# michaelriedl/2048-ppo-agent

Hardware: AMD Instinct MI355X
Metric: env-steps/sec at N parallel boards (full PPO loop: rollout with policy in the loop + GAE + update) (higher is better)
Workload: dtype u8 boards / bf16 policy; 1 GPU; 65536 parallel boards per GPU, Transformer policy bf16 (3.96 M params), full PPO iteration (BASELINE.json configs[2]; configs[3] when n_gpus=8); boards_per_gpu=65536, global_boards=65536, train_batch=2048, update_epochs=5, max_samples_per_epoch=300000, max_samples_per_epoch_is=global (each rank draws its 1/N share), as the reference's single subset, max_samples_per_epoch_per_rank=300000, rollout_mode=episodes (reference lock-step semantics), rng_mode=partitionable, parallelism=env-shard x1 + 1 grad all-reduce/minibatch

## Files before the change

2048-ppo-agent_amd/csrc/g2048_policy.hip:

```cpp
#include <hip/hip_runtime.h>
#include <stddef.h>
#include <stdint.h>
#include <stdlib.h>

#include "../../include/g2048.h"
#include "g2048_host.h"
#include "g2048_mfma.h"

namespace {

using g2048_mfma::bf16x4;
using g2048_mfma::bf16x8;
using g2048_mfma::f32x16;
using g2048_mfma::f32x4;
using g2048_mfma::mfma;
using g2048_mfma::rowof;
using g2048_mfma::sched_fence;
using g2048_mfma::static_for;
using namespace g2048_host;

typedef short s16x2 __attribute__((ext_vector_type(2)));

constexpr int D = 256, NH = 8, HD = 32, FF = 1024, SEQ = 17, NBOARD = 7, NTOK = 128, THREADS = 256;
constexpr int W_LAYER = 3 * D * D + D * D + FF * D + D * FF;
constexpr int P_LAYER = D + D + 3 * D + D + D + D + FF + D;
constexpr int WO_QKV = 0, WO_O = 3 * D * D, WO_1 = WO_O + D * D, WO_2 = WO_1 + FF * D;
constexpr int PO_LN1G = 0, PO_LN1B = D, PO_BQKV = 2 * D, PO_BO = 5 * D, PO_LN2G = 6 * D, PO_LN2B = 7 * D,
              PO_B1 = 8 * D, PO_B2 = 8 * D + FF;
constexpr int FFC = 64;
constexpr int TILE = 32 * D * 2;
constexpr float SM_SCALE_LOG2E = 0.17677669529663687f * 1.4426950408889634f;

template <int CPR> __device__ __forceinline__ int swz(int r);
template <> __device__ __forceinline__ int swz<32>(int r) { return r & 15; }
template <> __device__ __forceinline__ int swz<16>(int r) { return r & 15; }
template <> __device__ __forceinline__ int swz<8>(int r) { return (r >> 1) & 7; }
template <> __device__ __forceinline__ int swz<4>(int r) { return (r >> 2) & 3; }

struct LaneOff {
    int a256[8];
    int a64[4];
    int a32[2];
    unsigned s256[2], s64, s32;
};
__device__ __forceinline__ void lane_offsets(LaneOff &o, int r, int h, int w, int lane) {
    for (int k = 0; k < 8; ++k) o.a256[k] = r * 512 + (((2 * k + h) ^ swz<32>(r)) * 16);
    for (int k = 0; k < 4; ++k) o.a64[k] = r * 128 + (((2 * k + h) ^ swz<8>(r)) * 16);
    for (int k = 0; k < 2; ++k) o.a32[k] = r * 64 + (((2 * k + h) ^ swz<4>(r)) * 16);
    for (int par = 0; par < 2; ++par) {
        const int x = 2 * w + (lane >> 5), row15 = (8 * par + x) & 15;
        o.s256[par] = (unsigned)(x * D * 2 + (((lane & 31) ^ row15) * 16));
    }
    {
        const int x = 8 * w + (lane >> 3);
        o.s64 = (unsigned)(x * FF * 2 + (((lane & 7) ^ swz<8>(x)) * 16));
    }
    {
        const int x = 16 * w + (lane >> 2);
        o.s32 = (unsigned)(x * D * 2 + (((lane & 3) ^ swz<4>(x)) * 16));
    }
}

template <int CPR>
__device__ __forceinline__ bf16x8 load_w(const char *tile, const LaneOff &o, int mt, int ks) {
    if (CPR == 32) return *reinterpret_cast<const bf16x8 *>(tile + o.a256[ks & 7] + (ks >> 3) * 256 + mt * 32 * 512);
    if (CPR == 8) return *reinterpret_cast<const bf16x8 *>(tile + o.a64[ks] + mt * 32 * 128);
    return *reinterpret_cast<const bf16x8 *>(tile + o.a32[ks] + mt * 32 * 64);
}
__device__ __forceinline__ bf16x8 load_p(const char *row, int ks, int h) {
    return *reinterpret_cast<const bf16x8 *>(row + 2 * (16 * ks + 8 * h));
}

__device__ __forceinline__ void frag_from_acc(const f32x16 &x, bf16x8 out[2]) {
    for (int s = 0; s < 2; ++s)
        for (int j = 0; j < 8; ++j) out[s][j] = (__bf16)x[8 * s + j];
}
__device__ __forceinline__ void relu_frag_from_acc(const f32x16 &x, bf16x8 out[2]) {
    frag_from_acc(x, out);
    for (int s = 0; s < 2; ++s) {
        s16x2 *p = reinterpret_cast<s16x2 *>(&out[s]);
        const s16x2 zero = {0, 0};
        for (int q = 0; q < 4; ++q) p[q] = __builtin_elementwise_max(p[q], zero);
    }
}

__device__ __forceinline__ f32x16 bias_tile(const float *b32, int h) {
    f32x16 a;
    for (int g = 0; g < 4; ++g) {
        const f32x4 v = *reinterpret_cast<const f32x4 *>(b32 + 8 * g + 4 * h);
        for (int q = 0; q < 4; ++q) a[4 * g + q] = v[q];
    }
    return a;
}

template <int CPR, int NK, bool SWAP = false>
__device__ __forceinline__ f32x16 gemm_tile(const char *tile, const LaneOff &o, int mt, const bf16x8 *b, f32x16 acc) {
    bf16x8 a[NK];
    for (int ks = 0; ks < NK; ++ks) a[ks] = load_w<CPR>(tile, o, mt, ks);
    for (int ks = 0; ks < NK; ++ks) acc = SWAP ? mfma(b[ks], a[ks], acc) : mfma(a[ks], b[ks], acc);
    return acc;
}
template <int NM, int EXTRA = 0, int NV = 0, int VALU_PER = 0, int TRANS_PER = 0, int DEPTH = 8>
__device__ __forceinline__ void pipe_mfma() {
    __builtin_amdgcn_sched_group_barrier(0x100, DEPTH + EXTRA, 0);
#pragma unroll
    for (int i = 0; i < NM; ++i) {
        __builtin_amdgcn_sched_group_barrier(0x008, 1, 0);
        if (i < NM - DEPTH) __builtin_amdgcn_sched_group_barrier(0x100, 1, 0);
        if (i < NV && VALU_PER) __builtin_amdgcn_sched_group_barrier(0x002, VALU_PER, 0);
        if (i < NV && TRANS_PER) __builtin_amdgcn_sched_group_barrier(0x400, TRANS_PER, 0);
    }
}

#ifdef G2048_STAMPS
constexpr int N_STAMPS = 24;
__device__ unsigned long long g_stamps[N_STAMPS];
struct StampSite {
    __device__ __forceinline__ static bool on(int lane, int w) { return lane == 0 && w == 0 && blockIdx.x % 64 == 0; }
    __device__ __forceinline__ static unsigned long long *table(int) { return g_stamps; }
};
#define STAMP(k) stamps.mark(k)
#else
#define STAMP(k)
#endif

typedef __amdgpu_buffer_rsrc_t rsrc_t;
template <int CPR>
__device__ __forceinline__ void dma_tile(char *dst, rsrc_t blob, unsigned src_byte, int ld, int rows, const LaneOff &o, int w) {
    const int n_inst = rows * CPR / (64 * 4);
    const int rows_per_inst = 4 * 64 / CPR;
    for (int t = 0; t < n_inst; ++t) {
        const unsigned lane_off = CPR == 32 ? o.s256[t & 1] : (CPR == 8 ? o.s64 : o.s32);
        __builtin_amdgcn_raw_ptr_buffer_load_lds(blob, (__attribute__((address_space(3))) void *)(dst + (t * 4 + w) * 1024), 16,
                                                 (int)lane_off, (int)(src_byte + (unsigned)(t * rows_per_inst * ld * 2)), 0, 0);
    }
}
template <int CPR>
__device__ __forceinline__ void dma_inst(char *dst, rsrc_t blob, unsigned src_byte, int ld, int t, const LaneOff &o, int w) {
    const int rows_per_inst = 4 * 64 / CPR;
    const unsigned lane_off = CPR == 32 ? o.s256[t & 1] : (CPR == 8 ? o.s64 : o.s32);
    __builtin_amdgcn_raw_ptr_buffer_load_lds(blob, (__attribute__((address_space(3))) void *)(dst + (t * 4 + w) * 1024), 16,
                                             (int)lane_off, (int)(src_byte + (unsigned)(t * rows_per_inst * ld * 2)), 0, 0);
}
template <int N> __device__ __forceinline__ void dma_wait() { asm volatile("s_waitcnt vmcnt(%0)" ::"n"(N) : "memory"); }
__device__ __forceinline__ void dma_wait_all() { dma_wait<0>(); }

__device__ __forceinline__ void stage_f32(float *dst, const float *src, int n, int tid) {
    for (int i = tid; i < n; i += THREADS) dst[i] = src[i];
}

__device__ __forceinline__ void park_in_agpr(bf16x8 &x) { asm volatile("" : "+a"(x)); }

__device__ __forceinline__ float xhalf_sum(float x) {
    const auto r = __builtin_amdgcn_permlane32_swap(__float_as_uint(x), __float_as_uint(x), false, false);
    return __uint_as_float(r[0]) + __uint_as_float(r[1]);
}
__device__ __forceinline__ float xhalf_max(float x) {
    const auto r = __builtin_amdgcn_permlane32_swap(__float_as_uint(x), __float_as_uint(x), false, false);
    return fmaxf(__uint_as_float(r[0]), __uint_as_float(r[1]));
}

__device__ __forceinline__ void layer_norm(const f32x16 r[8], bf16x8 out[16]) {
    typedef float f32x2 __attribute__((ext_vector_type(2)));
    f32x2 s2[4], q2[4];
    for (int k = 0; k < 4; ++k) s2[k] = q2[k] = f32x2{0.f, 0.f};
    for (int j = 0; j < 8; ++j)
        for (int i = 0; i < 16; i += 2) {
            const f32x2 v = {r[j][i], r[j][i + 1]};
            const int k = (i >> 1) & 3;
            s2[k] += v;
            q2[k] = __builtin_elementwise_fma(v, v, q2[k]);
        }
    const f32x2 st = (s2[0] + s2[1]) + (s2[2] + s2[3]), qt = (q2[0] + q2[1]) + (q2[2] + q2[3]);
    float s = st[0] + st[1], ss = qt[0] + qt[1];
    s = xhalf_sum(s);
    ss = xhalf_sum(ss);
    const float mean = s * (1.0f / D);
    const float var = fmaxf(__builtin_fmaf(-mean, mean, ss * (1.0f / D)), 0.0f);
    const float rstd = rsqrtf(var + 1e-5f), shift = -mean * rstd;
    for (int j = 0; j < 8; ++j)
        for (int i = 0; i < 16; ++i) out[2 * j + (i >> 3)][i & 7] = (__bf16)__builtin_fmaf(r[j][i], rstd, shift);
    for (int k = 0; k < 16; ++k) park_in_agpr(out[k]);
}

constexpr int MODE_FULL = 0, MODE_HEAD = 1, MODE_MEAN = 2, MODE_CLS = 3;
constexpr int64_t KV_ELEMS = (int64_t)NH * SEQ * HD;

constexpr int L_WQKV = 0;
constexpr int L_WO = 6 * TILE;
constexpr int L_K = 7 * TILE;
constexpr int L_VT = 7 * TILE + TILE / 2;
constexpr int L_W1 = 0;
constexpr int L_W2 = 4 * TILE;
constexpr int L_CX = 6 * TILE;
constexpr int L_CQ = L_CX + 4096;
constexpr int L_CS = L_CQ + 1024;
constexpr int L_CO = L_CS + 1280;
constexpr int L_CV = 7 * TILE;
static_assert(L_CO + (NBOARD + 1) * D * 2 <= L_CV && L_CV + 2 * NTOK * HD * 2 <= 8 * TILE, "CLS staging fits the free tiles");
struct LdsMain {
    char w[8 * TILE];
    float bq[D], bo[D], b1[FF], b2[D];
};
static_assert(sizeof(LdsMain) <= 160 * 1024, "LDS budget");
constexpr int MEAN_LD = D + 4;
static_assert(NBOARD * 16 * MEAN_LD * 4 <= (int)sizeof(LdsMain::w), "mean-pool stage fits over the weight area");

template <int MODE>
__global__ void __launch_bounds__(THREADS, 1)
k_encoder_main(const uint8_t *__restrict__ boards, const float *__restrict__ table, const float *__restrict__ cls,
               const __bf16 *__restrict__ wblob, const float *__restrict__ pblob, int n_layers,
               float *__restrict__ features, int64_t B, __bf16 *__restrict__ ws_k, __bf16 *__restrict__ ws_v,
               float *__restrict__ ws_r) {
    extern __shared__ __attribute__((aligned(16))) char smem[];
    LdsMain &L = *reinterpret_cast<LdsMain *>(smem);
    const int tid = threadIdx.x, lane = tid & 63, r = lane & 31, h = lane >> 5;
    const int w = __builtin_amdgcn_readfirstlane(tid >> 6);
    const int64_t board0 = (int64_t)blockIdx.x * NBOARD;
    LaneOff lo;
    lane_offsets(lo, r, h, w, lane);

    const int tok = 32 * w + r;
    const int tb = tok / SEQ;
    const int tc = tok - tb * SEQ;
    const bool tok_valid = tb < NBOARD && board0 + tb < B;

    const int kb = w == 0 ? 0 : (w == 1 ? 16 : (w == 2 ? 48 : 64));
    int k_rd[2], vt_rd[4], k_wr[2], vt_wr[2];
    for (int ks = 0; ks < 2; ++ks) k_rd[ks] = L_K + kb * 64 + lo.a32[ks];
    for (int ks = 0; ks < 4; ++ks) vt_rd[ks] = L_VT + r * 256 + (((kb / 8 + 2 * ks + h) ^ swz<16>(r)) * 16);
    for (int s = 0; s < 2; ++s) {
        k_wr[s] = L_K + tok * 64 + (((2 * s + h) ^ swz<4>(tok)) * 16);
        vt_wr[s] = L_VT + r * 256 + (((4 * w + 2 * s + h) ^ swz<16>(r)) * 16);
    }
    bf16x8 kmask[2], qmask;
    {
        const int qb = tb;
        for (int j = 0; j < 8; ++j) qmask[j] = (__bf16)((qb == 8 * h + j) ? 16.0f : 0.0f);
        for (int tl = 0; tl < 2; ++tl) {
            const int kbd = (kb + 32 * tl + r) / SEQ;
            for (int j = 0; j < 8; ++j) kmask[tl][j] = (__bf16)((kbd == 8 * h + j) ? 16.0f : 0.0f);
        }
        park_in_agpr(qmask);
        park_in_agpr(kmask[0]);
        park_in_agpr(kmask[1]);
    }

    f32x16 R[8];
    {
        const float *src = cls;
        if (tok_valid && tc != 0) {
            int e = boards[(board0 + tb) * 16 + (tc - 1)];
            e = e > 30 ? 30 : e;
            src = table + ((size_t)(tc - 1) * 31 + e) * D;
        }
        const float keep = tok_valid ? 1.0f : 0.0f;
        for (int j = 0; j < 8; ++j)
            for (int g = 0; g < 4; ++g) {
                const f32x4 v = *reinterpret_cast<const f32x4 *>(src + 32 * j + 8 * g + 4 * h);
                for (int q = 0; q < 4; ++q) R[j][4 * g + q] = keep * v[q];
            }
    }

    const int full_layers = (MODE == MODE_HEAD || MODE == MODE_CLS) ? n_layers - 1 : n_layers;
    char *const lds = L.w;
    const rsrc_t blob = __builtin_amdgcn_make_buffer_rsrc(const_cast<__bf16 *>(wblob), 0, n_layers * (W_LAYER * 2), 0x00020000);
    auto wqkv = [&](int hd) -> char * { return lds + L_WQKV + (hd & 1) * 3 * TILE; };
    auto dma_qkv1 = [&](unsigned lw, int hd, int n) __attribute__((always_inline)) {
        dma_inst<32>(wqkv(hd) + (n / 4) * TILE, blob, lw + 2u * (unsigned)(WO_QKV + ((n / 4) * D + HD * hd) * D), D, n % 4, lo, w);
    };
    auto dma_wo1 = [&](unsigned lw, int hd, int n) __attribute__((always_inline)) {
        dma_inst<4>(lds + L_WO, blob, lw + 2u * (unsigned)(WO_O + HD * hd), D, n, lo, w);
    };
    auto dma_w11 = [&](unsigned lw, int c, int n) __attribute__((always_inline)) {
        dma_inst<32>(lds + L_W1 + (c & 1) * 2 * TILE, blob, lw + 2u * (unsigned)(WO_1 + FFC * c * D), D, n, lo, w);
    };
    auto dma_w21 = [&](unsigned lw, int c, int n) __attribute__((always_inline)) {
        dma_inst<8>(lds + L_W2 + (c & 1) * 2 * TILE, blob, lw + 2u * (unsigned)(WO_2 + FFC * c), FF, n, lo, w);
    };

#ifdef G2048_STAMPS
    g2048_mfma::Stamps<N_STAMPS, StampSite> stamps;
    stamps.start();
#endif
    for (int n = 0; n < 12; ++n) dma_qkv1(0u, 0, n);
    for (int n = 0; n < 12; ++n) dma_qkv1(0u, 1, n);

    constexpr int PD = 8;
    bf16x8 xn[16];
#pragma nounroll
    for (int layer = 0; layer < full_layers; ++layer) {
        const unsigned lw = (unsigned)layer * (unsigned)(W_LAYER * 2);
        const float *P = pblob + (size_t)layer * P_LAYER;

        float stg[7];
        stg[0] = P[PO_BQKV + tid];
        stg[1] = P[PO_BO + tid];
        stg[2] = P[PO_B2 + tid];
        for (int q = 0; q < 4; ++q) stg[3 + q] = P[PO_B1 + 256 * q + tid];
        layer_norm(R, xn);
        L.bq[tid] = stg[0];
        L.bo[tid] = stg[1];
        L.b2[tid] = stg[2];
        for (int q = 0; q < 4; ++q) L.b1[256 * q + tid] = stg[3 + q];
        dma_wait_all();
        __syncthreads();
        STAMP(0);

        f32x16 qa, ka, va;
        bf16x8 qf[2], kf[2], vf[2];
        auto project = [&](int hd, auto softmax_tag, auto fetch, f32x16 &s0, f32x16 &s1, bf16x8 *pf, float &sum) __attribute__((always_inline)) {
            constexpr bool SOFTMAX = decltype(softmax_tag)::value;
            const char *t = wqkv(hd);
            bf16x8 a[PD];
            qa = bias_tile(L.bq + HD * hd, h);
            for (int i = 0; i < 16; ++i) ka[i] = va[i] = 0.f;
            static_for<0, PD>([&](auto ic) __attribute__((always_inline)) {
                constexpr int i = decltype(ic)::value;
                a[i] = load_w<32>(t + (i / 16) * TILE, lo, 0, i % 16);
            });
            float m = 0.f, mc = 0.f;
            sched_fence();
            static_for<0, 48>([&](auto ic) __attribute__((always_inline)) {
                constexpr int i = decltype(ic)::value;
                constexpr int ks = i % 16;
                if constexpr (i < 16) qa = mfma(a[i % PD], xn[ks], qa);
                else if constexpr (i < 32) ka = mfma(a[i % PD], xn[ks], ka);
                else va = mfma(xn[ks], a[i % PD], va);
                if constexpr (i + PD < 48) a[i % PD] = load_w<32>(t + ((i + PD) / 16) * TILE, lo, 0, (i + PD) % 16);
                if constexpr (i % 3 == 0) fetch(std::integral_constant<int, i / 3>{});
                if constexpr (SOFTMAX) {
                    if constexpr (i < 8) {
                        const float x = fmaxf(fmaxf(s0[2 * i], s0[2 * i + 1]), fmaxf(s1[2 * i], s1[2 * i + 1]));
                        m = i == 0 ? x : fmaxf(m, x);
                    } else if constexpr (i == 8) {
                        m = xhalf_max(m);
                        mc = -m * SM_SCALE_LOG2E;
                        sum = 0.f;
                    } else if constexpr (i < 41) {
                        constexpr int e = i - 9;
                        if constexpr (e < 16) {
                            s0[e] = __builtin_amdgcn_exp2f(__builtin_fmaf(s0[e], SM_SCALE_LOG2E, mc));
                            sum += s0[e];
                        } else {
                            s1[e - 16] = __builtin_amdgcn_exp2f(__builtin_fmaf(s1[e - 16], SM_SCALE_LOG2E, mc));
                            sum += s1[e - 16];
                        }
                    } else if constexpr (i == 41) {
                        sum = xhalf_sum(sum);
                    } else if constexpr (i < 46) {
                        constexpr int k = i - 42;
                        for (int j = 0; j < 8; ++j) {
                            if constexpr (k < 2) pf[k][j] = (__bf16)s0[8 * (k & 1) + j];
                            else pf[k][j] = (__bf16)s1[8 * (k & 1) + j];
                        }
                    }
                }
                sched_fence();
            });
        };
        auto pack_qkv = [&](auto nc) __attribute__((always_inline)) {
            constexpr int n = decltype(nc)::value, which = n / 4, s = (n / 2) & 1, half = n & 1;
            for (int j = 0; j < 4; ++j) {
                if constexpr (which == 0) qf[s][4 * half + j] = (__bf16)qa[8 * s + 4 * half + j];
                else if constexpr (which == 1) kf[s][4 * half + j] = (__bf16)ka[8 * s + 4 * half + j];
                else vf[s][4 * half + j] = (__bf16)va[8 * s + 4 * half + j];
            }
        };
        auto store_kv = [&]() __attribute__((always_inline)) {
            for (int s = 0; s < 2; ++s) {
                *reinterpret_cast<bf16x8 *>(lds + k_wr[s]) = kf[s];
                *reinterpret_cast<bf16x8 *>(lds + vt_wr[s]) = vf[s];
            }
        };
        {
            f32x16 d0, d1;
            float dsum;
            project(0, std::false_type{}, [](auto) {}, d0, d1, nullptr, dsum);
            static_for<0, 12>(pack_qkv);
        }
        store_kv();
        __syncthreads();
        STAMP(1);

        auto head = [&](int hd, auto next_tag) __attribute__((always_inline)) {
            constexpr int NEXT = decltype(next_tag)::value;
            bf16x8 kr[4];
            for (int ks = 0; ks < 2; ++ks) {
                kr[2 * ks] = *reinterpret_cast<const bf16x8 *>(lds + k_rd[ks]);
                kr[2 * ks + 1] = *reinterpret_cast<const bf16x8 *>(lds + k_rd[ks] + 32 * 64);
            }
            sched_fence();
            auto fetch = [&](auto nc) __attribute__((always_inline)) {
                constexpr int n = decltype(nc)::value;
                if constexpr (n < 4) dma_wo1(lw, hd, n);
                else if constexpr (NEXT == 0) dma_qkv1(lw, hd + 2, n - 4);
                else if constexpr (NEXT == 1 && n < 12) dma_w11(lw, 0, n - 4);
            };
            if constexpr (NEXT == 2) static_for<0, 4>(fetch);
            sched_fence();
            STAMP(2);
            f32x16 s0 = {0}, s1 = {0};
            for (int ks = 0; ks < 2; ++ks) {
                s0 = mfma(kr[2 * ks], qf[ks], s0);
                s1 = mfma(kr[2 * ks + 1], qf[ks], s1);
            }
            s0 = mfma(kmask[0], qmask, s0);
            s1 = mfma(kmask[1], qmask, s1);
            sched_fence();
            STAMP(3);
            bf16x8 pf[4];
            float sum;
            if constexpr (NEXT != 2) {
                project(hd + 1, std::true_type{}, fetch, s0, s1, pf, sum);
            } else {
                float m = fmaxf(s0[0], s1[0]);
                for (int i = 1; i < 16; ++i) m = fmaxf(m, fmaxf(s0[i], s1[i]));
                m = xhalf_max(m);
                const float mc = -m * SM_SCALE_LOG2E;
                sum = 0.f;
                for (int i = 0; i < 16; ++i) {
                    s0[i] = __builtin_amdgcn_exp2f(__builtin_fmaf(s0[i], SM_SCALE_LOG2E, mc));
                    s1[i] = __builtin_amdgcn_exp2f(__builtin_fmaf(s1[i], SM_SCALE_LOG2E, mc));
                    sum += s0[i] + s1[i];
                }
                sum = xhalf_sum(sum);
                frag_from_acc(s0, pf);
                frag_from_acc(s1, pf + 2);
            }
            sched_fence();
            STAMP(4);
            f32x16 o = {0};
            for (int ks = 0; ks < 4; ++ks) o = mfma(*reinterpret_cast<const bf16x8 *>(lds + vt_rd[ks]), pf[ks], o);
            const float inv = __builtin_amdgcn_rcpf(sum);
            for (int i = 0; i < 16; ++i) o[i] *= inv;
            bf16x8 of[2];
            frag_from_acc(o, of);
            STAMP(5);
            if constexpr (NEXT == 0) dma_wait<12>();
            if constexpr (NEXT == 1) dma_wait<8>();
            if constexpr (NEXT == 2) dma_wait<0>();
            asm volatile("s_waitcnt lgkmcnt(0)" ::: "memory");
            __builtin_amdgcn_s_barrier();
            sched_fence();
            STAMP(6);
            {
                const char *wo = lds + L_WO;
                bf16x8 a[PD];
                static_for<0, PD>([&](auto ic) __attribute__((always_inline)) {
                    constexpr int i = decltype(ic)::value;
                    a[i] = load_w<4>(wo, lo, i / 2, i % 2);
                });
                sched_fence();
                static_for<0, 16>([&](auto ic) __attribute__((always_inline)) {
                    constexpr int i = decltype(ic)::value;
                    R[i / 2] = mfma(a[i % PD], of[i % 2], R[i / 2]);
                    if constexpr (i + PD < 16) a[i % PD] = load_w<4>(wo, lo, (i + PD) / 2, (i + PD) % 2);
                    if constexpr (NEXT != 2 && i < 12) pack_qkv(ic);
                    if constexpr (NEXT != 2 && i == 12) store_kv();
                    sched_fence();
                });
            }
            STAMP(7);
            dma_wait_all();
            STAMP(8);
            __syncthreads();
            STAMP(9);
        };
#pragma nounroll
        for (int hd = 0; hd < NH - 2; ++hd) head(hd, std::integral_constant<int, 0>{});
        head(NH - 2, std::integral_constant<int, 1>{});
        head(NH - 1, std::integral_constant<int, 2>{});

        for (int j = 0; j < 8; ++j) {
            dma_w11(lw, 1, j);
            const f32x16 b = bias_tile(L.bo + 32 * j, h);
            for (int i = 0; i < 16; ++i) R[j][i] += b[i];
        }
        layer_norm(R, xn);
        STAMP(10);
        f32x16 hA0, hA1, hB0, hB1;
        bf16x8 hf[4];
        auto pack_h = [&](auto nc, const f32x16 &g0, const f32x16 &g1) __attribute__((always_inline)) {
            constexpr int n = decltype(nc)::value, k = n / 4, q = n % 4;
            for (int j = 0; j < 2; ++j) {
                if constexpr (k < 2) hf[k][2 * q + j] = (__bf16)g0[8 * (k & 1) + 2 * q + j];
                else hf[k][2 * q + j] = (__bf16)g1[8 * (k & 1) + 2 * q + j];
            }
            if constexpr (q == 3) {
                s16x2 *p2 = reinterpret_cast<s16x2 *>(&hf[k]);
                const s16x2 zero = {0, 0};
                for (int u = 0; u < 4; ++u) p2[u] = __builtin_elementwise_max(p2[u], zero);
            }
        };
        auto ffn_chain = [&](auto with1_tag, auto with2_tag, int c1, int c2, f32x16 &n0, f32x16 &n1, const f32x16 &g0, const f32x16 &g1,
                             auto fetch) __attribute__((always_inline)) {
            constexpr bool WITH1 = decltype(with1_tag)::value, WITH2 = decltype(with2_tag)::value;
            constexpr int N1 = WITH1 ? 32 : 0, NS = N1 + (WITH2 ? 32 : 0);
            const char *t1 = lds + L_W1 + (c1 & 1) * 2 * TILE, *t2 = lds + L_W2 + (c2 & 1) * 2 * TILE;
            if constexpr (WITH1) {
                n0 = bias_tile(L.b1 + FFC * c1, h);
                n1 = bias_tile(L.b1 + FFC * c1 + 32, h);
            }
            bf16x8 a[PD];
            auto rd = [&](auto sc) __attribute__((always_inline)) {
                constexpr int s = decltype(sc)::value;
                if constexpr (s < N1) a[s % PD] = load_w<32>(t1, lo, s / 16, s % 16);
                else a[s % PD] = load_w<8>(t2, lo, (s - N1) / 4, (s - N1) % 4);
            };
            static_for<0, PD>(rd);
            if constexpr (!WITH1 && WITH2) static_for<0, 16>([&](auto nc) __attribute__((always_inline)) { pack_h(nc, g0, g1); });
            sched_fence();
            static_for<0, NS>([&](auto ic) __attribute__((always_inline)) {
                constexpr int i = decltype(ic)::value;
                if constexpr (i < N1) {
                    if constexpr (i < 16) n0 = mfma(a[i % PD], xn[i % 16], n0);
                    else n1 = mfma(a[i % PD], xn[i % 16], n1);
                } else {
                    R[(i - N1) / 4] = mfma(a[i % PD], hf[(i - N1) % 4], R[(i - N1) / 4]);
                }
                if constexpr (i + PD < NS) rd(std::integral_constant<int, i + PD>{});
                if constexpr (NS == 64 ? (i % 3 == 0 && i < 48) : i % 2 == 0) fetch(std::integral_constant<int, NS == 64 ? i / 3 : i / 2>{});
                if constexpr (WITH1 && WITH2 && i < 16) pack_h(ic, g0, g1);
                sched_fence();
            });
        };
        {
            f32x16 dummy0, dummy1;
            ffn_chain(std::true_type{}, std::false_type{}, 0, 0, hA0, hA1, dummy0, dummy1, [&](auto nc) __attribute__((always_inline)) {
                constexpr int n = decltype(nc)::value;
                if constexpr (n < 8) dma_w21(lw, 0, n);
            });
        }
        dma_wait_all();
        __syncthreads();
        STAMP(11);
        auto chunk = [&](int c, auto last_tag, f32x16 &n0, f32x16 &n1, const f32x16 &g0, const f32x16 &g1) __attribute__((always_inline)) {
            constexpr int LAST = decltype(last_tag)::value;
            auto fetch = [&](auto nc) __attribute__((always_inline)) {
                constexpr int n = decltype(nc)::value;
                if constexpr (LAST == 0) {
                    if constexpr (n < 8) dma_w11(lw, c + 2, n);
                    else dma_w21(lw, c + 1, n - 8);
                } else if constexpr (LAST == 1) {
                    if constexpr (n < 8) dma_w21(lw, c + 1, n);
                    else dma_qkv1(lw + W_LAYER * 2, 0, n - 8);
                } else {
                    if constexpr (n < 4) dma_qkv1(lw + W_LAYER * 2, 0, 8 + n);
                    else dma_qkv1(lw + W_LAYER * 2, 1, n - 4);
                }
            };
            STAMP(12);
            if constexpr (LAST != 2) ffn_chain(std::true_type{}, std::true_type{}, c + 1, c, n0, n1, g0, g1, fetch);
            else ffn_chain(std::false_type{}, std::true_type{}, 0, c, n0, n1, g0, g1, fetch);
            STAMP(14);
            if constexpr (LAST == 2)
                for (int j = 0; j < 8; ++j) {
                    const f32x16 b = bias_tile(L.b2 + 32 * j, h);
                    for (int i = 0; i < 16; ++i) R[j][i] += b[i];
                }
            dma_wait_all();
            STAMP(15);
            __syncthreads();
            STAMP(16);
        };
#pragma nounroll
        for (int c = 0; c < FF / FFC - 2; c += 2) {
            chunk(c, std::integral_constant<int, 0>{}, hB0, hB1, hA0, hA1);
            chunk(c + 1, std::integral_constant<int, 0>{}, hA0, hA1, hB0, hB1);
        }
        chunk(FF / FFC - 2, std::integral_constant<int, 1>{}, hB0, hB1, hA0, hA1);
        chunk(FF / FFC - 1, std::integral_constant<int, 2>{}, hA0, hA1, hB0, hB1);
    }

    STAMP(17);
    if (MODE == MODE_HEAD) {
        const unsigned lwl = (unsigned)(n_layers - 1) * (unsigned)(W_LAYER * 2);
        if (tok_valid && tc == 0) {
            float *dst = ws_r + (board0 + tb) * D;
            for (int j = 0; j < 8; ++j)
                for (int g = 0; g < 4; ++g) {
                    f32x4 v;
                    for (int q = 0; q < 4; ++q) v[q] = R[j][4 * g + q];
                    *reinterpret_cast<f32x4 *>(dst + 32 * j + 8 * g + 4 * h) = v;
                }
        }
        layer_norm(R, xn);
        dma_wait_all();
        __syncthreads();
        bf16x8 kst[2], vst[2];
        auto store_head = [&](int hd) __attribute__((always_inline)) {
            if (tok_valid) {
                const size_t off = (size_t)(board0 + tb) * KV_ELEMS + ((size_t)hd * SEQ + tc) * HD + 16 * h;
                *reinterpret_cast<bf16x8 *>(ws_k + off) = kst[0];
                *reinterpret_cast<bf16x8 *>(ws_k + off + 8) = kst[1];
                *reinterpret_cast<bf16x8 *>(ws_v + off) = vst[0];
                *reinterpret_cast<bf16x8 *>(ws_v + off + 8) = vst[1];
            }
        };
        auto kv_head = [&](int hd, auto fetch_tag, auto store_tag) __attribute__((always_inline)) {
            constexpr bool FETCH = decltype(fetch_tag)::value, STORE = decltype(store_tag)::value;
            if constexpr (STORE) store_head(hd - 1);
            const char *t = wqkv(hd);
            f32x16 ka2 = {0}, va2 = {0};
            bf16x8 a[PD];
            static_for<0, PD>([&](auto ic) __attribute__((always_inline)) {
                constexpr int i = decltype(ic)::value;
                a[i] = load_w<32>(t + (1 + i / 16) * TILE, lo, 0, i % 16);
            });
            sched_fence();
            static_for<0, 32>([&](auto ic) __attribute__((always_inline)) {
                constexpr int i = decltype(ic)::value;
                if constexpr (i < 16) ka2 = mfma(a[i % PD], xn[i % 16], ka2);
                else va2 = mfma(a[i % PD], xn[i % 16], va2);
                if constexpr (i + PD < 32) a[i % PD] = load_w<32>(t + (1 + (i + PD) / 16) * TILE, lo, 0, (i + PD) % 16);
                if constexpr (FETCH && i % 3 == 0 && i < 24) dma_qkv1(lwl, hd + 1, 4 + i / 3);
                if constexpr (i >= 20 && i < 22)
                    for (int j = 0; j < 8; ++j) kst[i - 20][j] = (__bf16)ka2[8 * (i - 20) + j];
                sched_fence();
            });
            frag_from_acc(va2, vst);
            dma_wait_all();
            __syncthreads();
        };
        kv_head(0, std::false_type{}, std::false_type{});
#pragma nounroll
        for (int hd = 1; hd < NH - 1; ++hd) kv_head(hd, std::true_type{}, std::true_type{});
        kv_head(NH - 1, std::false_type{}, std::true_type{});
        store_head(NH - 1);
        STAMP(18);
#ifdef G2048_STAMPS
        stamps.flush(lane, w);
#endif
        return;
    }

    if constexpr (MODE == MODE_CLS) {
        const unsigned lwl = (unsigned)(n_layers - 1) * (unsigned)(W_LAYER * 2);
        const float bq_stage = pblob[(size_t)(n_layers - 1) * P_LAYER + PO_BQKV + tid];
        __bf16 *const ws_o = ws_k;
        if (tok_valid && tc == 0) {
            float *dst = ws_r + (board0 + tb) * D;
            for (int j = 0; j < 8; ++j)
                for (int g = 0; g < 4; ++g) {
                    f32x4 v;
                    for (int q = 0; q < 4; ++q) v[q] = R[j][4 * g + q];
                    *reinterpret_cast<f32x4 *>(dst + 32 * j + 8 * g + 4 * h) = v;
                }
        }
        layer_norm(R, xn);
        L.bq[tid] = bq_stage;
        if (tb < NBOARD && tc == 0)
            for (int ks = 0; ks < 16; ++ks) *reinterpret_cast<bf16x8 *>(lds + L_CX + ((2 * ks + h) * 8 + tb) * 16) = xn[ks];
        dma_wait_all();
        __syncthreads();
        const int sb = 2 * w + h;
        const int sbc = sb < NBOARD ? sb : 0;
        bf16x8 kst[2], vst[2];
        constexpr std::true_type yes{};
        constexpr std::false_type no{};
        auto cls_head = [&](int it, auto kv_tag, auto fetch_tag, auto score_tag, auto soft_tag) __attribute__((always_inline)) {
            constexpr bool KV = decltype(kv_tag)::value, FETCH = decltype(fetch_tag)::value;
            constexpr bool SCORE = decltype(score_tag)::value, SOFT = decltype(soft_tag)::value;
            const int pb = (it - 1) & 1, sbuf = it & 1;
            bf16x8 q0, q1;
            float d = 0.f, scv[SEQ], m = -3.0e38f, sum = 0.f, o = 0.f;
            __bf16 vv[SEQ];
            if constexpr (SCORE) {
                q0 = *reinterpret_cast<const bf16x8 *>(lds + L_CQ + pb * 512 + tb * 64 + h * 32);
                q1 = *reinterpret_cast<const bf16x8 *>(lds + L_CQ + pb * 512 + tb * 64 + h * 32 + 16);
            }
            if constexpr (SOFT) {
                const char *src = lds + L_CS + (sbuf * 160 + sbc * 20) * 4;
                for (int g = 0; g < 4; ++g) {
                    const f32x4 v = *reinterpret_cast<const f32x4 *>(src + 16 * g);
                    for (int q = 0; q < 4; ++q) scv[4 * g + q] = v[q];
                }
                scv[16] = *reinterpret_cast<const float *>(src + 64);
            }
            auto piece = [&](auto ic) __attribute__((always_inline)) {
                constexpr int i = decltype(ic)::value;
                if constexpr (SCORE) {
                    if constexpr (i == 0) {
                        for (int s = 0; s < 2; ++s)
                            *reinterpret_cast<bf16x8 *>(lds + L_CV + pb * (NTOK * HD * 2) + tok * (HD * 2) + (16 * s + 8 * h) * 2) = vst[s];
                    }
                    if constexpr (i < 8) {
                        d += (float)q0[i] * (float)kst[0][i] + (float)q1[i] * (float)kst[1][i];
                    } else if constexpr (i == 8) {
                        d = xhalf_sum(d);
                        *reinterpret_cast<float *>(lds + L_CS + (pb * 160 + tb * 20 + tc) * 4) = d * 0.17677669529663687f;
                    }
                }
                if constexpr (SOFT) {
                    if constexpr (i < SEQ)
                        vv[i] = *reinterpret_cast<const __bf16 *>(lds + L_CV + sbuf * (NTOK * HD * 2) + (SEQ * sbc + i) * (HD * 2) + r * 2);
                    if constexpr (i == 9) {
                        for (int key = 0; key < SEQ; ++key) m = fmaxf(m, scv[key]);
                    } else if constexpr (i >= 10 && i < 10 + SEQ) {
                        constexpr int key = i - 10;
                        scv[key] = __expf(scv[key] - m);
                        sum += scv[key];
                        const float p = (float)(__bf16)scv[key];
                        o += p * (float)vv[key];
                    } else if constexpr (i == 10 + SEQ) {
                        const float inv = 1.0f / sum;
                        *reinterpret_cast<__bf16 *>(lds + L_CO + sb * (D * 2) + ((it - 2) * HD + r) * 2) = (__bf16)(o * inv);
                    }
                }
            };
            if constexpr (KV) {
                auto chain = [&](auto qw_tag) __attribute__((always_inline)) {
                    constexpr bool QW = decltype(qw_tag)::value;
                    constexpr int NQ = QW ? 16 : 0, NS = NQ + 32;
                    const char *t = wqkv(it);
                    const char *xsrc = lds + L_CX + (h * 8 + (r & 7)) * 16;
                    f32x16 ka2 = {0}, va2 = {0}, qa = {0};
                    if constexpr (QW) qa = bias_tile(L.bq + HD * it, h);
                    bf16x8 a[PD], bx[PD];
                    auto rd = [&](auto sc) __attribute__((always_inline)) {
                        constexpr int s = decltype(sc)::value;
                        if constexpr (s < NQ) {
                            a[s % PD] = load_w<32>(t, lo, 0, s);
                            bx[s % PD] = *reinterpret_cast<const bf16x8 *>(xsrc + s * 256);
                        } else {
                            a[s % PD] = load_w<32>(t + (1 + (s - NQ) / 16) * TILE, lo, 0, (s - NQ) % 16);
                        }
                    };
                    static_for<0, PD>(rd);
                    sched_fence();
                    static_for<0, NS>([&](auto ic) __attribute__((always_inline)) {
                        constexpr int i = decltype(ic)::value, j = i - NQ;
                        if constexpr (i < NQ) qa = mfma(a[i % PD], bx[i % PD], qa);
                        else if constexpr (j < 16) ka2 = mfma(a[i % PD], xn[j], ka2);
                        else va2 = mfma(a[i % PD], xn[j - 16], va2);
                        if constexpr (i + PD < NS) rd(std::integral_constant<int, i + PD>{});
                        if constexpr (FETCH && i % 2 == 0 && i < 24) dma_qkv1(lwl, it + 1, i / 2);
                        if constexpr (i < 32) piece(ic);
                        if constexpr (j >= 20 && j < 22)
                            for (int e = 0; e < 8; ++e) kst[j - 20][e] = (__bf16)ka2[8 * (j - 20) + e];
                        sched_fence();
                    });
                    frag_from_acc(va2, vst);
                    if constexpr (QW) {
                        if (r < NBOARD)
                            for (int s = 0; s < 2; ++s) {
                                bf16x8 qv;
                                for (int e = 0; e < 8; ++e) qv[e] = (__bf16)qa[8 * s + e];
                                *reinterpret_cast<bf16x8 *>(lds + L_CQ + (it & 1) * 512 + r * 64 + h * 32 + 16 * s) = qv;
                            }
                    }
                };
                if (w == (it & 3)) chain(yes);
                else chain(no);
            } else {
                static_for<0, 32>(piece);
            }
            dma_wait_all();
            __syncthreads();
        };
        cls_head(0, yes, no, no, no);
        cls_head(1, yes, yes, yes, no);
#pragma nounroll
        for (int it = 2; it < NH - 1; ++it) cls_head(it, yes, yes, yes, yes);
        cls_head(NH - 1, yes, no, yes, yes);
        cls_head(NH, no, no, yes, yes);
        cls_head(NH + 1, no, no, no, yes);
        if (tid < NBOARD * 32 && board0 + (tid >> 5) < B)
            *reinterpret_cast<bf16x8 *>(ws_o + (board0 + (tid >> 5)) * D + (tid & 31) * 8) =
                *reinterpret_cast<const bf16x8 *>(lds + L_CO + (tid >> 5) * (D * 2) + (tid & 31) * 16);
        STAMP(18);
#ifdef G2048_STAMPS
        stamps.flush(lane, w);
#endif
        return;
    }

    if constexpr (MODE == MODE_MEAN) {
        dma_wait_all();
        __syncthreads();
        const int ln = (int)__builtin_amdgcn_mbcnt_hi(~0u, __builtin_amdgcn_mbcnt_lo(~0u, 0u));
        const int t = 64 * w + ln, mtok = 32 * w + (ln & 31), mtb = mtok / SEQ, mtc = mtok - mtb * SEQ, mh = ln >> 5;
        float *const stage = reinterpret_cast<float *>(lds);
        if (mtb < NBOARD && board0 + mtb < B && mtc != 0) {
            float *dst = stage + (mtb * 16 + mtc - 1) * MEAN_LD;
            for (int j = 0; j < 8; ++j)
                for (int g = 0; g < 4; ++g) {
                    f32x4 v;
                    for (int q = 0; q < 4; ++q) v[q] = R[j][4 * g + q];
                    *reinterpret_cast<f32x4 *>(dst + 32 * j + 8 * g + 4 * mh) = v;
                }
        }
        __syncthreads();
        for (int b = 0; b < NBOARD && board0 + b < B; ++b) {
            const float *src = stage + b * 16 * MEAN_LD + t;
            float s = 0.f;
            for (int k = 0; k < 16; ++k) s += src[k * MEAN_LD];
            features[(board0 + b) * D + t] = s * 0.0625f;
        }
    } else {
        if (tok_valid && tc == 0) {
            float *dst = features + (board0 + tb) * D;
            for (int j = 0; j < 8; ++j)
                for (int g = 0; g < 4; ++g) {
                    f32x4 v;
                    for (int q = 0; q < 4; ++q) v[q] = R[j][4 * g + q];
                    *reinterpret_cast<f32x4 *>(dst + 32 * j + 8 * g + 4 * h) = v;
                }
        }
    }
}

constexpr int ST32 = 2 * 32 + 16;
struct LdsTail {
    char w[6 * TILE];
    char w2b[2 * TILE];
    char o[NTOK * ST32];
    float bias[FF];
};
static_assert(sizeof(LdsTail) <= 160 * 1024, "LDS budget");
static_assert(offsetof(LdsTail, w2b) == 6 * TILE, "w and w2b are one 8-tile area (the whole out_proj.weight)");

template <bool KVWS>
__global__ void __launch_bounds__(THREADS, 1)
k_encoder_tail(const __bf16 *__restrict__ wblob, const float *__restrict__ pblob, int n_layers, float *__restrict__ features,
               int64_t B, const __bf16 *__restrict__ ws_k, const __bf16 *__restrict__ ws_v, const float *__restrict__ ws_r) {
    extern __shared__ __attribute__((aligned(16))) char smem[];
    LdsTail &L = *reinterpret_cast<LdsTail *>(smem);
    const int tid = threadIdx.x, lane = tid & 63, r = lane & 31, h = lane >> 5;
    const int w = __builtin_amdgcn_readfirstlane(tid >> 6);
    const int64_t board0 = (int64_t)blockIdx.x * NTOK;
    char *const wq = L.w;
    LaneOff lo;
    lane_offsets(lo, r, h, w, lane);
    const int tok = 32 * w + r;
    const bool tok_valid = board0 + tok < B;
    const int64_t my_board = tok_valid ? board0 + tok : (B - 1);

    f32x16 R[8];
    {
        const float *src = ws_r + my_board * D;
        for (int j = 0; j < 8; ++j)
            for (int g = 0; g < 4; ++g) {
                const f32x4 v = *reinterpret_cast<const f32x4 *>(src + 32 * j + 8 * g + 4 * h);
                for (int q = 0; q < 4; ++q) R[j][4 * g + q] = v[q];
            }
    }
    const rsrc_t blob = __builtin_amdgcn_make_buffer_rsrc(const_cast<__bf16 *>(wblob), 0, n_layers * (W_LAYER * 2), 0x00020000);
    const unsigned lw = (unsigned)(n_layers - 1) * (unsigned)(W_LAYER * 2);
    const float *P = pblob + (size_t)(n_layers - 1) * P_LAYER;
    auto dma_q = [&](int hd) { dma_tile<32>(wq, blob, lw + 2u * (unsigned)(WO_QKV + HD * hd * D), D, HD, lo, w); };
    auto wo_of = [&](int hd) -> char * { return L.w + (3 + (hd & 1)) * TILE; };
    auto dma_wo = [&](int hd) { dma_tile<4>(wo_of(hd), blob, lw + 2u * (unsigned)(WO_O + HD * hd), D, D, lo, w); };

    bf16x8 xn[16];
    if constexpr (!KVWS) {
        for (int hd = 0; hd < NH; ++hd) dma_tile<4>(L.w + hd * TILE, blob, lw + 2u * (unsigned)(WO_O + HD * hd), D, D, lo, w);
        bf16x8 of[NH][2];
        for (int hd = 0; hd < NH; ++hd)
            for (int ks = 0; ks < 2; ++ks) of[hd][ks] = *reinterpret_cast<const bf16x8 *>(ws_k + my_board * D + hd * HD + 16 * ks + 8 * h);
        dma_wait_all();
        __syncthreads();
#pragma unroll
        for (int hd = 0; hd < NH; ++hd)
            for (int j = 0; j < 8; ++j) R[j] = gemm_tile<4, 2>(L.w + hd * TILE, lo, j, of[hd], R[j]);
        pipe_mfma<16 * NH>();
        __syncthreads();
    }
    if constexpr (KVWS) {
    dma_q(0);
    dma_wo(0);
    stage_f32(L.bias, P + PO_BQKV, D, tid);
    layer_norm(R, xn);
    dma_wait_all();
    __syncthreads();
#pragma nounroll
    for (int hd = 0; hd < NH; ++hd) {
        f32x16 qa = gemm_tile<32, 16>(wq, lo, 0, xn, bias_tile(L.bias + HD * hd, h));
        pipe_mfma<16>();
        const size_t off = (size_t)my_board * KV_ELEMS + (size_t)hd * SEQ * HD + 16 * h;
        float sc[SEQ], m = -3.0e38f;
        for (int key = 0; key < SEQ; ++key) {
            const bf16x8 k0 = *reinterpret_cast<const bf16x8 *>(ws_k + off + key * HD);
            const bf16x8 k1 = *reinterpret_cast<const bf16x8 *>(ws_k + off + key * HD + 8);
            float d = 0.f;
            for (int i = 0; i < 8; ++i) d += (float)(__bf16)qa[i] * (float)k0[i] + (float)(__bf16)qa[8 + i] * (float)k1[i];
            d = xhalf_sum(d);
            sc[key] = d * 0.17677669529663687f;
            m = fmaxf(m, sc[key]);
        }
        float sum = 0.f;
        for (int key = 0; key < SEQ; ++key) {
            sc[key] = __expf(sc[key] - m);
            sum += sc[key];
        }
        const float inv = 1.0f / sum;
        float o[16];
        for (int i = 0; i < 16; ++i) o[i] = 0.f;
        for (int key = 0; key < SEQ; ++key) {
            const bf16x8 v0 = *reinterpret_cast<const bf16x8 *>(ws_v + off + key * HD);
            const bf16x8 v1 = *reinterpret_cast<const bf16x8 *>(ws_v + off + key * HD + 8);
            const float p = (float)(__bf16)sc[key];
            for (int i = 0; i < 8; ++i) {
                o[i] += p * (float)v0[i];
                o[8 + i] += p * (float)v1[i];
            }
        }
        for (int s = 0; s < 2; ++s) {
            bf16x8 ov;
            for (int q = 0; q < 8; ++q) ov[q] = (__bf16)(o[8 * s + q] * inv);
            *reinterpret_cast<bf16x8 *>(L.o + tok * ST32 + 2 * (16 * s + 8 * h)) = ov;
        }
        __syncthreads();
        if (hd + 1 < NH) {
            dma_q(hd + 1);
            dma_wo(hd + 1);
        }
        bf16x8 of[2];
        for (int ks = 0; ks < 2; ++ks) of[ks] = load_p(L.o + tok * ST32, ks, h);
        const char *wo = wo_of(hd);
        for (int j = 0; j < 8; ++j) R[j] = gemm_tile<4, 2>(wo, lo, j, of, R[j]);
        pipe_mfma<16>();
        dma_wait_all();
        __syncthreads();
    }
    }

    auto w1_of = [&](int c) -> char * { return L.w + ((c & 1) ? 2 * TILE : 0); };
    auto w2_of = [&](int c) -> char * { return (c & 1) ? L.w2b : L.w + 4 * TILE; };
    auto dma_ffn = [&](int c) {
        dma_tile<32>(w1_of(c), blob, lw + 2u * (unsigned)(WO_1 + FFC * c * D), D, FFC, lo, w);
        dma_tile<8>(w2_of(c), blob, lw + 2u * (unsigned)(WO_2 + FFC * c), FF, D, lo, w);
    };
    dma_ffn(0);
    stage_f32(L.bias, P + PO_BO, D, tid);
    __syncthreads();
    for (int j = 0; j < 8; ++j) {
        const f32x16 b = bias_tile(L.bias + 32 * j, h);
        for (int i = 0; i < 16; ++i) R[j][i] += b[i];
    }
    layer_norm(R, xn);
    __syncthreads();
    stage_f32(L.bias, P + PO_B1, FF, tid);
    dma_wait_all();
    __syncthreads();
#pragma nounroll
    for (int c = 0; c < FF / FFC; ++c) {
        if (c + 1 < FF / FFC) dma_ffn(c + 1);
        const char *t1 = w1_of(c), *t2 = w2_of(c);
        f32x16 h0 = gemm_tile<32, 16>(t1, lo, 0, xn, bias_tile(L.bias + FFC * c, h));
        f32x16 h1 = gemm_tile<32, 16>(t1, lo, 1, xn, bias_tile(L.bias + FFC * c + 32, h));
        pipe_mfma<32>();
        bf16x8 hf[4];
        relu_frag_from_acc(h0, hf);
        relu_frag_from_acc(h1, hf + 2);
        for (int j = 0; j < 8; ++j) R[j] = gemm_tile<8, 4>(t2, lo, j, hf, R[j]);
        pipe_mfma<32>();
        dma_wait_all();
        __syncthreads();
    }
    if (tok_valid) {
        float *dst = features + (board0 + tok) * D;
        for (int j = 0; j < 8; ++j)
            for (int g = 0; g < 4; ++g) {
                const f32x4 b = *reinterpret_cast<const f32x4 *>(P + PO_B2 + 32 * j + 8 * g + 4 * h);
                f32x4 v;
                for (int q = 0; q < 4; ++q) v[q] = R[j][4 * g + q] + b[q];
                *reinterpret_cast<f32x4 *>(dst + 32 * j + 8 * g + 4 * h) = v;
            }
    }
}

}

#ifdef G2048_STAMPS
extern "C" int g2048_debug_stamps(unsigned long long *out , int reset) {
    if (hipMemcpyFromSymbol(out, HIP_SYMBOL(g_stamps), sizeof(unsigned long long) * N_STAMPS) != hipSuccess) return -1;
    if (reset) {
        unsigned long long z[N_STAMPS] = {0};
        if (hipMemcpyToSymbol(HIP_SYMBOL(g_stamps), z, sizeof(z)) != hipSuccess) return -1;
    }
    return N_STAMPS;
}
#endif

extern "C" int64_t g2048_policy_encoder_workspace_bytes(int64_t B) {
    return B <= 0 ? 0 : B * (2 * KV_ELEMS * (int64_t)sizeof(__bf16) + D * (int64_t)sizeof(float));
}

extern "C" int g2048_policy_encoder(const uint8_t *boards, const float *embed_table, const float *cls_token,
                                    const void *weights_bf16, const float *params_f32, int n_layers,
                                    float *features, int64_t B, void *workspace, void *stream) {
    if (!boards || !embed_table || !cls_token || !weights_bf16 || !params_f32 || !features || n_layers < 1 || B <= 0)
        return G2048_EINVAL;
    if (!aligned16(weights_bf16, params_f32, embed_table, cls_token, features, workspace)) return G2048_EINVAL;
    const char *e = getenv("G2048_ENCODER_KV_WS");
    const bool kv_ws = e && e[0] == '1';
    const void *main_fn = !workspace ? reinterpret_cast<const void *>(k_encoder_main<MODE_FULL>)
                          : kv_ws    ? reinterpret_cast<const void *>(k_encoder_main<MODE_HEAD>)
                                     : reinterpret_cast<const void *>(k_encoder_main<MODE_CLS>);
    const void *tail_fn = kv_ws ? reinterpret_cast<const void *>(k_encoder_tail<true>) : reinterpret_cast<const void *>(k_encoder_tail<false>);
    if (const int rc = allow_dynamic_lds(main_fn, (int)sizeof(LdsMain))) return rc;
    if (workspace)
        if (const int rc = allow_dynamic_lds(tail_fn, (int)sizeof(LdsTail))) return rc;
    const __bf16 *wb = reinterpret_cast<const __bf16 *>(weights_bf16);
    const unsigned blocks = (unsigned)((B + NBOARD - 1) / NBOARD);
    if (!workspace) {
        hipLaunchKernelGGL(k_encoder_main<MODE_FULL>, dim3(blocks), dim3(THREADS), sizeof(LdsMain), (hipStream_t)stream, boards,
                           embed_table, cls_token, wb, params_f32, n_layers, features, B, (__bf16 *)nullptr, (__bf16 *)nullptr,
                           (float *)nullptr);
    } else if (!kv_ws) {
        __bf16 *ws_o = reinterpret_cast<__bf16 *>(workspace);
        float *ws_r = reinterpret_cast<float *>(ws_o + B * D);
        hipLaunchKernelGGL(k_encoder_main<MODE_CLS>, dim3(blocks), dim3(THREADS), sizeof(LdsMain), (hipStream_t)stream, boards,
                           embed_table, cls_token, wb, params_f32, n_layers, features, B, ws_o, (__bf16 *)nullptr, ws_r);
        hipLaunchKernelGGL(k_encoder_tail<false>, dim3((unsigned)((B + NTOK - 1) / NTOK)), dim3(THREADS), sizeof(LdsTail),
                           (hipStream_t)stream, wb, params_f32, n_layers, features, B, (const __bf16 *)ws_o, (const __bf16 *)nullptr,
                           (const float *)ws_r);
    } else {
        __bf16 *ws_k = reinterpret_cast<__bf16 *>(workspace), *ws_v = ws_k + B * KV_ELEMS;
        float *ws_r = reinterpret_cast<float *>(ws_v + B * KV_ELEMS);
        hipLaunchKernelGGL(k_encoder_main<MODE_HEAD>, dim3(blocks), dim3(THREADS), sizeof(LdsMain), (hipStream_t)stream, boards,
                           embed_table, cls_token, wb, params_f32, n_layers, features, B, ws_k, ws_v, ws_r);
        hipLaunchKernelGGL(k_encoder_tail<true>, dim3((unsigned)((B + NTOK - 1) / NTOK)), dim3(THREADS), sizeof(LdsTail),
                           (hipStream_t)stream, wb, params_f32, n_layers, features, B, ws_k, ws_v, ws_r);
    }
    return launch_status();
}

extern "C" int g2048_policy_encoder_mean(const uint8_t *boards, const float *embed_table, const float *cls_token,
                                         const void *weights_bf16, const float *params_f32, int n_layers, float *features,
                                         int64_t B, void *stream) {
    if (!boards || !embed_table || !cls_token || !weights_bf16 || !params_f32 || !features || n_layers < 1 || B <= 0)
        return G2048_EINVAL;
    if (!aligned16(weights_bf16, params_f32, embed_table, cls_token, features)) return G2048_EINVAL;
    if (const int rc = allow_dynamic_lds(reinterpret_cast<const void *>(k_encoder_main<MODE_MEAN>), (int)sizeof(LdsMain))) return rc;
    const unsigned blocks = (unsigned)((B + NBOARD - 1) / NBOARD);
    hipLaunchKernelGGL(k_encoder_main<MODE_MEAN>, dim3(blocks), dim3(THREADS), sizeof(LdsMain), (hipStream_t)stream, boards,
                       embed_table, cls_token, reinterpret_cast<const __bf16 *>(weights_bf16), params_f32, n_layers, features, B,
                       (__bf16 *)nullptr, (__bf16 *)nullptr, (float *)nullptr);
    return launch_status();
}
```

Before: 3.881 million env-steps/sec.

## Interleave softmax, bf16 packing and output scaling with MFMA chains in attention

Reschedules the attention head's softmax so the max reduction is spread over more MFMA steps. The exp stage now packs probabilities to bf16 pairs inline, and the reciprocal of the sum is computed inside the projection chain. QKV packing is moved into the PV and output-projection MFMA loops, with the O-projection loop order changed. Conversions use paired bf16x2 vector converts, and some accumulators are pinned to AGPRs/VGPRs via asm constraints. The intent is to hide VALU conversion and softmax work behind matrix instructions, at the cost of more register pressure and fragile scheduling.

```diff
diff --git a/2048-ppo-agent_amd/csrc/g2048_policy.hip b/2048-ppo-agent_amd/csrc/g2048_policy.hip
--- a/2048-ppo-agent_amd/csrc/g2048_policy.hip
+++ b/2048-ppo-agent_amd/csrc/g2048_policy.hip
@@ -20,6 +20,8 @@
 using namespace g2048_host;
 
 typedef short s16x2 __attribute__((ext_vector_type(2)));
+typedef float f32x2 __attribute__((ext_vector_type(2)));
+typedef __bf16 bf16x2 __attribute__((ext_vector_type(2)));
 
 constexpr int D = 256, NH = 8, HD = 32, FF = 1024, SEQ = 17, NBOARD = 7, NTOK = 128, THREADS = 256;
 constexpr int W_LAYER = 3 * D * D + D * D + FF * D + D * FF;
@@ -150,6 +152,8 @@
 }
 
 __device__ __forceinline__ void park_in_agpr(bf16x8 &x) { asm volatile("" : "+a"(x)); }
+
+template <class T> __device__ __forceinline__ void pin_in_vgpr(T &x) { asm volatile("" : "+v"(x)); }
 
 __device__ __forceinline__ float xhalf_sum(float x) {
     const auto r = __builtin_amdgcn_permlane32_swap(__float_as_uint(x), __float_as_uint(x), false, false);
@@ -309,8 +313,9 @@
 
         f32x16 qa, ka, va;
         bf16x8 qf[2], kf[2], vf[2];
-        auto project = [&](int hd, auto softmax_tag, auto fetch, f32x16 &s0, f32x16 &s1, bf16x8 *pf, float &sum) __attribute__((always_inline)) {
+        auto project = [&](int hd, auto softmax_tag, auto fetch, f32x16 &s0, f32x16 &s1, bf16x8 *pf, float &inv) __attribute__((always_inline)) {
             constexpr bool SOFTMAX = decltype(softmax_tag)::value;
+            constexpr int MAX_STEPS = 13;
             const char *t = wqkv(hd);
             bf16x8 a[PD];
             qa = bias_tile(L.bq + HD * hd, h);
@@ -319,7 +324,7 @@
                 constexpr int i = decltype(ic)::value;
                 a[i] = load_w<32>(t + (i / 16) * TILE, lo, 0, i % 16);
             });
-            float m = 0.f, mc = 0.f;
+            float m = 0.f, mc = 0.f, sum = 0.f;
             sched_fence();
             static_for<0, 48>([&](auto ic) __attribute__((always_inline)) {
                 constexpr int i = decltype(ic)::value;
@@ -330,42 +335,46 @@
                 if constexpr (i + PD < 48) a[i % PD] = load_w<32>(t + ((i + PD) / 16) * TILE, lo, 0, (i + PD) % 16);
                 if constexpr (i % 3 == 0) fetch(std::integral_constant<int, i / 3>{});
                 if constexpr (SOFTMAX) {
-                    if constexpr (i < 8) {
-                        const float x = fmaxf(fmaxf(s0[2 * i], s0[2 * i + 1]), fmaxf(s1[2 * i], s1[2 * i + 1]));
-                        m = i == 0 ? x : fmaxf(m, x);
-                    } else if constexpr (i == 8) {
+                    auto sc = [&](auto ec) __attribute__((always_inline)) -> float {
+                        constexpr int e = decltype(ec)::value;
+                        if constexpr (e < 16) return s0[e];
+                        else return s1[e - 16];
+                    };
+                    if constexpr (i < MAX_STEPS) {
+                        constexpr int e0 = i < 6 ? 3 * i : 2 * i + 6, n = i < 6 ? 3 : 2;
+                        static_for<0, n>([&](auto jc) __attribute__((always_inline)) {
+                            const float x = sc(std::integral_constant<int, e0 + decltype(jc)::value>{});
+                            m = (i == 0 && decltype(jc)::value == 0) ? x : fmaxf(m, x);
+                        });
+                    } else if constexpr (i == MAX_STEPS) {
                         m = xhalf_max(m);
                         mc = -m * SM_SCALE_LOG2E;
-                        sum = 0.f;
-                    } else if constexpr (i < 41) {
-                        constexpr int e = i - 9;
-                        if constexpr (e < 16) {
-                            s0[e] = __builtin_amdgcn_exp2f(__builtin_fmaf(s0[e], SM_SCALE_LOG2E, mc));
-                            sum += s0[e];
-                        } else {
-                            s1[e - 16] = __builtin_amdgcn_exp2f(__builtin_fmaf(s1[e - 16], SM_SCALE_LOG2E, mc));
-                            sum += s1[e - 16];
+                    } else if constexpr (i <= MAX_STEPS + 32) {
+                        constexpr int e = i - MAX_STEPS - 1;
+                        const float p = __builtin_amdgcn_exp2f(__builtin_fmaf(sc(std::integral_constant<int, e>{}), SM_SCALE_LOG2E, mc));
+                        sum += p;
+                        if constexpr (e < 16) s0[e] = p;
+                        else s1[e - 16] = p;
+                        if constexpr (e % 2 == 1) {
+                            const f32x2 v = {sc(std::integral_constant<int, e - 1>{}), p};
+                            uint32_t pr = __builtin_bit_cast(uint32_t, __builtin_convertvector(v, bf16x2));
+                            pin_in_vgpr(pr);
+                            reinterpret_cast<uint32_t *>(&pf[e / 8])[(e % 8) / 2] = pr;
                         }
-                    } else if constexpr (i == 41) {
-                        sum = xhalf_sum(sum);
-                    } else if constexpr (i < 46) {
-                        constexpr int k = i - 42;
-                        for (int j = 0; j < 8; ++j) {
-                            if constexpr (k < 2) pf[k][j] = (__bf16)s0[8 * (k & 1) + j];
-                            else pf[k][j] = (__bf16)s1[8 * (k & 1) + j];
-                        }
+                    } else if constexpr (i == MAX_STEPS + 33) {
+                        inv = __builtin_amdgcn_rcpf(xhalf_sum(sum));
+                        pin_in_vgpr(inv);
                     }
                 }
                 sched_fence();
             });
         };
         auto pack_qkv = [&](auto nc) __attribute__((always_inline)) {
-            constexpr int n = decltype(nc)::value, which = n / 4, s = (n / 2) & 1, half = n & 1;
-            for (int j = 0; j < 4; ++j) {
-                if constexpr (which == 0) qf[s][4 * half + j] = (__bf16)qa[8 * s + 4 * half + j];
-                else if constexpr (which == 1) kf[s][4 * half + j] = (__bf16)ka[8 * s + 4 * half + j];
-                else vf[s][4 * half + j] = (__bf16)va[8 * s + 4 * half + j];
-            }
+            constexpr int n = decltype(nc)::value, which = n / 8, s = (n / 4) & 1, pr = n & 3;
+            const f32x16 &x = which == 0 ? qa : (which == 1 ? ka : va);
+            bf16x8 &f = which == 0 ? qf[s] : (which == 1 ? kf[s] : vf[s]);
+            const f32x2 v = {x[8 * s + 2 * pr], x[8 * s + 2 * pr + 1]};
+            reinterpret_cast<bf16x2 *>(&f)[pr] = __builtin_convertvector(v, bf16x2);
         };
         auto store_kv = [&]() __attribute__((always_inline)) {
             for (int s = 0; s < 2; ++s) {
@@ -375,9 +384,9 @@
         };
         {
             f32x16 d0, d1;
-            float dsum;
-            project(0, std::false_type{}, [](auto) {}, d0, d1, nullptr, dsum);
-            static_for<0, 12>(pack_qkv);
+            float dinv;
+            project(0, std::false_type{}, [](auto) {}, d0, d1, nullptr, dinv);
+            static_for<0, 24>(pack_qkv);
         }
         store_kv();
         __syncthreads();
@@ -410,32 +419,48 @@
             sched_fence();
             STAMP(3);
             bf16x8 pf[4];
-            float sum;
+            float inv;
             if constexpr (NEXT != 2) {
-                project(hd + 1, std::true_type{}, fetch, s0, s1, pf, sum);
+                project(hd + 1, std::true_type{}, fetch, s0, s1, pf, inv);
             } else {
                 float m = fmaxf(s0[0], s1[0]);
                 for (int i = 1; i < 16; ++i) m = fmaxf(m, fmaxf(s0[i], s1[i]));
                 m = xhalf_max(m);
                 const float mc = -m * SM_SCALE_LOG2E;
-                sum = 0.f;
+                float sum = 0.f;
                 for (int i = 0; i < 16; ++i) {
                     s0[i] = __builtin_amdgcn_exp2f(__builtin_fmaf(s0[i], SM_SCALE_LOG2E, mc));
                     s1[i] = __builtin_amdgcn_exp2f(__builtin_fmaf(s1[i], SM_SCALE_LOG2E, mc));
                     sum += s0[i] + s1[i];
                 }
-                sum = xhalf_sum(sum);
+                inv = __builtin_amdgcn_rcpf(xhalf_sum(sum));
                 frag_from_acc(s0, pf);
                 frag_from_acc(s1, pf + 2);
             }
             sched_fence();
             STAMP(4);
             f32x16 o = {0};
-            for (int ks = 0; ks < 4; ++ks) o = mfma(*reinterpret_cast<const bf16x8 *>(lds + vt_rd[ks]), pf[ks], o);
-            const float inv = __builtin_amdgcn_rcpf(sum);
-            for (int i = 0; i < 16; ++i) o[i] *= inv;
+            {
+                bf16x8 vt[4];
+                for (int ks = 0; ks < 4; ++ks) vt[ks] = *reinterpret_cast<const bf16x8 *>(lds + vt_rd[ks]);
+                sched_fence();
+                static_for<0, 4>([&](auto kc) __attribute__((always_inline)) {
+                    constexpr int ks = decltype(kc)::value;
+                    o = mfma(vt[ks], pf[ks], o);
+                    if constexpr (NEXT != 2) {
+                        pack_qkv(std::integral_constant<int, 2 * ks>{});
+                        pack_qkv(std::integral_constant<int, 2 * ks + 1>{});
+                    }
+                    sched_fence();
+                });
+            }
             bf16x8 of[2];
-            frag_from_acc(o, of);
+            auto scale_o = [&](auto pc) __attribute__((always_inline)) {
+                constexpr int p = decltype(pc)::value;
+                const f32x2 v = {o[2 * p] * inv, o[2 * p + 1] * inv};
+                reinterpret_cast<bf16x2 *>(&of[p / 4])[p % 4] = __builtin_convertvector(v, bf16x2);
+            };
+            static_for<0, 4>(scale_o);
             STAMP(5);
             if constexpr (NEXT == 0) dma_wait<12>();
             if constexpr (NEXT == 1) dma_wait<8>();
@@ -443,23 +468,25 @@
             asm volatile("s_waitcnt lgkmcnt(0)" ::: "memory");
             __builtin_amdgcn_s_barrier();
             sched_fence();
+            asm volatile("" : "+a"(o));
             STAMP(6);
             {
                 const char *wo = lds + L_WO;
                 bf16x8 a[PD];
                 static_for<0, PD>([&](auto ic) __attribute__((always_inline)) {
                     constexpr int i = decltype(ic)::value;
-                    a[i] = load_w<4>(wo, lo, i / 2, i % 2);
+                    a[i] = load_w<4>(wo, lo, i % 8, i / 8);
                 });
                 sched_fence();
                 static_for<0, 16>([&](auto ic) __attribute__((always_inline)) {
                     constexpr int i = decltype(ic)::value;
-                    R[i / 2] = mfma(a[i % PD], of[i % 2], R[i / 2]);
-                    if constexpr (i + PD < 16) a[i % PD] = load_w<4>(wo, lo, (i + PD) / 2, (i + PD) % 2);
-                    if constexpr (NEXT != 2 && i < 12) pack_qkv(ic);
-                    if constexpr (NEXT != 2 && i == 12) store_kv();
+                    R[i % 8] = mfma(a[i % PD], of[i / 8], R[i % 8]);
+                    if constexpr (i + PD < 16) a[i % PD] = load_w<4>(wo, lo, (i + PD) % 8, (i + PD) / 8);
+                    if constexpr (i % 2 == 1 && i < 8) scale_o(std::integral_constant<int, 4 + i / 2>{});
+                    if constexpr (NEXT != 2) pack_qkv(std::integral_constant<int, 8 + i>{});
                     sched_fence();
                 });
+                if constexpr (NEXT != 2) store_kv();
             }
             STAMP(7);
             dma_wait_all();
@@ -483,15 +510,10 @@
         bf16x8 hf[4];
         auto pack_h = [&](auto nc, const f32x16 &g0, const f32x16 &g1) __attribute__((always_inline)) {
             constexpr int n = decltype(nc)::value, k = n / 4, q = n % 4;
-            for (int j = 0; j < 2; ++j) {
-                if constexpr (k < 2) hf[k][2 * q + j] = (__bf16)g0[8 * (k & 1) + 2 * q + j];
-                else hf[k][2 * q + j] = (__bf16)g1[8 * (k & 1) + 2 * q + j];
-            }
-            if constexpr (q == 3) {
-                s16x2 *p2 = reinterpret_cast<s16x2 *>(&hf[k]);
-                const s16x2 zero = {0, 0};
-                for (int u = 0; u < 4; ++u) p2[u] = __builtin_elementwise_max(p2[u], zero);
-            }
+            const f32x16 &g = k < 2 ? g0 : g1;
+            const f32x2 v = {g[8 * (k & 1) + 2 * q], g[8 * (k & 1) + 2 * q + 1]};
+            const s16x2 zero = {0, 0};
+            reinterpret_cast<s16x2 *>(&hf[k])[q] = __builtin_elementwise_max(__builtin_bit_cast(s16x2, __builtin_convertvector(v, bf16x2)), zero);
         };
         auto ffn_chain = [&](auto with1_tag, auto with2_tag, int c1, int c2, f32x16 &n0, f32x16 &n1, const f32x16 &g0, const f32x16 &g1,
                              auto fetch) __attribute__((always_inline)) {
@@ -511,6 +533,7 @@
             static_for<0, PD>(rd);
             if constexpr (!WITH1 && WITH2) static_for<0, 16>([&](auto nc) __attribute__((always_inline)) { pack_h(nc, g0, g1); });
             sched_fence();
+            if constexpr (WITH1 && WITH2) asm volatile("" : "+a"(const_cast<f32x16 &>(g0)), "+a"(const_cast<f32x16 &>(g1)));
             static_for<0, NS>([&](auto ic) __attribute__((always_inline)) {
                 constexpr int i = decltype(ic)::value;
                 if constexpr (i < N1) {
```

After: 3.919 million env-steps/sec, median of 6. No clear change (+1.0%).
